# Jiraiya812/Fast-CU-Decision-HEVC

Hardware: AMD Instinct MI355X
Metric: CTUs/sec (RDO decision only) at 4K all-intra (higher is better)
Workload: dtype int32+f64

## Files before the change

fast-cu-decision-hevc_amd/csrc/fcu_engine.h:

```cpp
#pragma once
#include <stdint.h>
#include <string.h>
#include <type_traits>
#include "../../include/fcu.h"

#ifdef FCU_EMU
#include <math.h>
#include <stdio.h>
#include <stdlib.h>
#define FCU_DEV static inline
#define FCU_MEMBER inline
#define FCU_NOINLINE
#define FCU_INLINE
#define FCU_TABLE static const
static int g_emu_phase = 0, g_emu_in_phase = 0, g_emu_lane = 0, g_emu_relax = 0;
#define FCU_EMU_RELAX(on) (g_emu_relax = (on))
static inline int fcu_emu_phase_begin() { g_emu_phase++; g_emu_in_phase = 1; g_emu_lane = 0; return 0; }
static inline int fcu_emu_phase_next(int lane) { if (lane + 1 >= 64) g_emu_in_phase = 0; g_emu_lane = lane + 1; return lane + 1; }
template <class T> static inline T fcu_emu_uni(T v, int site, int line)
{
  enum { SITES = 2048, K = 32, B = 16 };
  struct Seen { int phase, first, cur, idx, n; unsigned char vals[K][B]; };
  static Seen seen[SITES];
  if (g_emu_in_phase && !g_emu_relax && sizeof(T) <= B && site < SITES) {
// ... 75 lines not shown
#define FCU_DIST_ADD(acc, v, e, i, n2) do { \
    if ((n2) >= 64) { (acc) += (uint32_t)((e) * (e)); if (((((i) - lane) + 64) & ((n2) - 1)) == 0) { FCU_WAVE_ADD(&g_S.vc_dist[v], acc); (acc) = 0; } } \
    else FCU_ATOMIC_ADD(&g_S.vc_dist[v], (uint32_t)((e) * (e))); } while (0)
#define FCU_SERIAL FCU_FOR_LANES if (lane == 0)
#if defined(FCU_PROFILE) && !defined(FCU_EMU)
#define FCU_TIC(v) const long long v = clock64()
#ifdef FCU_PROFILE_RQT
#define FCU_QTIC(v) long long v = clock64()
#define FCU_QTOC(E_, v, idx) do { if (threadIdx.x == 0) (E_).C->prof[idx] += (unsigned long long)(clock64() - v); v = clock64(); } while (0)
#define FCU_TOC(E_, v, idx) do { if ((idx) == 10 && threadIdx.x == 0) (E_).C->prof[idx] += (unsigned long long)(clock64() - v); } while (0)
#define FCU_COUNT(E_, idx, n) do { } while (0)
#elif defined(FCU_PROFILE_INTER)
#define FCU_ITOC(E_, v, idx) do { if (threadIdx.x == 0) (E_).C->prof[idx] += (unsigned long long)(clock64() - v); } while (0)
#define FCU_TOC(E_, v, idx) do { if ((idx) == 10 && threadIdx.x == 0) (E_).C->prof[idx] += (unsigned long long)(clock64() - v); } while (0)
#define FCU_COUNT(E_, idx, n) do { } while (0)
#elif defined(FCU_PROFILE_RDOQ) || defined(FCU_PROFILE_DEPTH)
#define FCU_TOC(E_, v, idx) do { if ((idx) < 11 && threadIdx.x == 0) (E_).C->prof[idx] += (unsigned long long)(clock64() - v); } while (0)
#define FCU_COUNT(E_, idx, n) do { } while (0)
#elif defined(FCU_PROFILE_RMD)
#define FCU_MTOC(E_, v, idx) do { if (threadIdx.x == 0) (E_).C->prof[idx] += (unsigned long long)(clock64() - v); } while (0)
#define FCU_TOC(E_, v, idx) do { if ((idx) < 11 && threadIdx.x == 0) (E_).C->prof[idx] += (unsigned long long)(clock64() - v); } while (0)
#define FCU_COUNT(E_, idx, n) do { } while (0)
#elif defined(FCU_PROFILE_CUSYN)
#define FCU_STOC(E_, v, idx) do { if (threadIdx.x == 0) (E_).C->prof[idx] += (unsigned long long)(clock64() - v); } while (0)
#define FCU_SPATH(E_, path) do { if (threadIdx.x == 0) (E_).C->prof[15] += 1ull << (21 * (path)); } while (0)
#define FCU_S7_COEFF(E_, v, comp) do { if (g_S.prof_s7 == 1) FCU_STOC(E_, v, (comp) ? 14 : 13); } while (0)
#define FCU_TOC(E_, v, idx) do { if ((idx) < 11 && threadIdx.x == 0) (E_).C->prof[idx] += (unsigned long long)(clock64() - v); } while (0)
#define FCU_COUNT(E_, idx, n) do { } while (0)
#elif defined(FCU_PROFILE_PIX)
#define FCU_PTIC(v) long long v = clock64()
// ... 33 lines not shown
#endif

#include "fcu_tables.h"

struct HotTables { uint32_t bin[256]; uint16_t scan[3][16]; uint8_t scan_cg8[3][4]; uint8_t ctx_ind_map4x4[16]; uint8_t group_idx[32];
                   uint64_t scan4_nib[3], map4_nib; uint32_t cnt_bits[4]; };
#ifdef FCU_EMU
static HotTables g_hot;
#else
__shared__ HotTables g_hot;
#endif

#if defined(FCU_PROFILE_RQT) && !defined(FCU_EMU)
#define FCU_RTIC(v) long long v = clock64()
#define FCU_RTOC(P_, v, idx) do { if (!SER && threadIdx.x == 0) { ((Chain *)((char *)&(P_) - __builtin_offsetof(Chain, p)))->prof[idx] += (unsigned long long)(clock64() - v); v = clock64(); } } while (0)
#elif defined(FCU_PROFILE_RDOQ) && !defined(FCU_EMU)
#define FCU_RTIC(v) long long v = clock64()
#define FCU_RTOC(P_, v, idx) do { if ((FCU_PROFILE_RDOQ + 0) == 2 ? (!SER && threadIdx.x == 0) : SER) { ((Chain *)((char *)&(P_) - __builtin_offsetof(Chain, p)))->prof[idx] += (unsigned long long)(clock64() - v); v = clock64(); } } while (0)
#else
#define FCU_RTIC(v) do { } while (0)
#define FCU_RTOC(P_, v, idx) do { } while (0)
#endif
namespace fcu {

enum { CTU = 64, MAXDEPTH = 3, NPART = 256, LOG2_MAXTU = 5, LOG2_MINTU = 2, TU_MAXDEPTH_INTRA = 3 };
enum { SIZE_2Nx2N = 0, SIZE_2NxN = 1, SIZE_Nx2N = 2, SIZE_NxN = 3, SIZE_2NxnU = 4, SIZE_2NxnD = 5, SIZE_nLx2N = 6, SIZE_nRx2N = 7, SIZE_NONE = 8, MODE_INTER = 0, MODE_INTRA = 1, MODE_NONE = 2 };
enum { SLICE_I = 0, SLICE_P = 1 };
enum { PLANAR = 0, DC = 1, HOR = 10, VER = 26, DM_CHROMA = 36 };
enum { CTX_SPLIT = 0, CTX_PARTSIZE = 3, CTX_INTRA_LUMA = 4, CTX_CHROMA_PRED = 5, CTX_CBF_LUMA = 6, CTX_CBF_CHROMA = 11,
       CTX_SUBDIV = 16, CTX_SIGCG = 19, CTX_SIG = 23, CTX_LASTX = 67, CTX_LASTY = 97, CTX_ONE = 127, CTX_ABS = 151,
       CTX_TSKIP = 157, NCTX_INTRA = 160,
       CTX_SKIP = 160, CTX_MERGE_FLAG = 163, CTX_MERGE_IDX = 164, CTX_PRED_MODE = 165, CTX_PARTSIZE1 = 166, CTX_MVD = 169,
       CTX_REF = 171, CTX_MVP_IDX = 173, CTX_ROOT_CBF = 174, NCTX = 176 };
enum { CI_CURR_BEST = 0, CI_NEXT_BEST, CI_TEMP_BEST, CI_CHROMA_INTRA, CI_QT_TRAFO_TEST, CI_QT_TRAFO_ROOT, CI_NUM };
enum { MEMO_K = 6, MEMO_POOL = 6144 + 1536 + 384 + 96 };
enum { MAXVC = 20, MAXLC = 16, POOL = 5120 };
// ... 297 lines not shown
  return first + offset;
}
FCU_DEV int coef_remain_bins(uint32_t symbol, uint32_t rparam)
{
  int code = (int)symbol;
  if (code < (3 << rparam)) return (int)(((uint32_t)code >> rparam) + 1) + (int)rparam;
  uint32_t length = rparam;
  code -= 3 << rparam;
  while (code >= (1 << length)) code -= 1 << (length++);
  return (int)(3 + length + 1 - rparam) + (int)length;
}
#ifdef FCU_EMU
enum { WALK_RDOQ_CALLS, WALK_RDOQ_TOP_IS_GROUP0, WALK_RDOQ_AHEAD_GROUPS, WALK_RDOQ_ONLY_GROUP0, WALK_RDOQ_ONLY_LAST_GROUP, WALK_RDOQ_ALL_ZERO,
       WALK_BITS_CALLS, WALK_BITS_ONE_EMPTY_RUN_BETWEEN, WALK_BITS_SECOND_ROUND, WALK_N };
enum { SMALL_TS_WINNER, SMALL_ALL_ZERO, SMALL_BATCH_OVER_16, SMALL_CHROMA_4X4, SMALL_N };
extern "C" { __attribute__((weak)) unsigned long long fcu_emu_walk_cnt[WALK_N]; __attribute__((weak)) unsigned long long fcu_emu_small_cnt[SMALL_N]; }
#define FCU_SMALL_COUNT(i, n) (fcu_emu_small_cnt[i] += (unsigned long long)(n))
static const int32_t *g_emu_lscan_lo = nullptr, *g_emu_lscan_hi = nullptr;
#define FCU_WALK_COUNT(i, n) (fcu_emu_walk_cnt[i] += (unsigned long long)(n))
#define FCU_CHECK_LSCAN(p) FCU_CHECK((const int32_t *)(p) >= g_emu_lscan_lo && (const int32_t *)(p) < g_emu_lscan_hi)
#else
#define FCU_WALK_COUNT(i, n) do { } while (0)
#define FCU_SMALL_COUNT(i, n) do { } while (0)
#define FCU_CHECK_LSCAN(p) do { } while (0)
#endif
template <int SER>
FCU_DEV FCU_INLINE void code_coeff_body(int c, const int16_t *coef, int st, int last, int log2, int comp, int scanType, int tsFlag, const Params &P_, int16_t *absCoeff)
{
  if (SER) { c = FCU_UNI(c); coef = FCU_UNI(coef); last = FCU_UNI(last); scanType = FCU_UNI(scanType); tsFlag = FCU_UNI(tsFlag); absCoeff = FCU_UNI(absCoeff); }
  const Params &P = *FCU_UNI(&P_);
  st = FCU_UNI(st); log2 = FCU_UNI(log2); comp = FCU_UNI(comp);
  FCU_IN_LDS(absCoeff);
  const FCU_HBM int16_t *coefg = (const FCU_HBM int16_t *)coef;
  const int ch = comp ? 1 : 0, N = 1 << log2; int n2 = N * N;
  if (last < 0 && st == 1 && n2 >= 64) {
    int q = (n2 >> 6) - 1;
    for (; q >= 0; q--) {
      uint32_t w[32];
// ... 558 lines not shown
  }
#endif
  return rdoq_finish<SER>(cb, P, srcg, dstg, recg, cgg, st, log2, ch, scanType, cbfCtx, scan, scanCG, cgflag, cgLastScanPos, lastScanPos, baseCost, blockUncodedCost, lambda);
}

#ifdef FCU_EMU
template <class T> struct LaneVar {
  T v[64];
  LaneVar() { for (int i = 0; i < 64; i++) v[i] = T(); }
  void set(int lane, T x) { v[lane] = x; }
  T own(int lane) const { return v[lane]; }
  T get(int k) const { return v[k]; }
  void put(int k, T x) { v[k] = x; }
  T from(int src) const { return v[src & 63]; }
};
FCU_DEV uint32_t lane_mask16(const LaneVar<int> &f) { uint32_t m = 0; for (int k = 0; k < 16; k++) m |= (uint32_t)(f.v[k] != 0) << k; return m; }
#else
#if defined(__HIP_DEVICE_COMPILE__)
#define FCU_READLANE(v, k) __builtin_amdgcn_readlane((v), (k))
#define FCU_WRITELANE(val_, k_, old_) (((int)threadIdx.x == (k_)) ? (val_) : (old_))
#define FCU_BALLOT(p) __builtin_amdgcn_ballot_w64(p)
#define FCU_PERMUTE(v, src) __builtin_amdgcn_ds_bpermute((src) << 2, (v))
#else
#define FCU_READLANE(v, k) (v)
#define FCU_WRITELANE(val_, k_, old_) (val_)
#define FCU_BALLOT(p) ((unsigned long long)(p))
#define FCU_PERMUTE(v, src) (v)
#endif
template <class T> struct LaneVar;
template <> struct LaneVar<int> {
  int r = 0;
  __device__ void set(int, int x) { r = x; }
  __device__ int own(int) const { return r; }
  __device__ int get(int k) const { return FCU_READLANE(r, k); }
  __device__ void put(int k, int x) { r = FCU_WRITELANE(x, k, r); }
  __device__ int from(int src) const { return FCU_PERMUTE(r, src); }
};
template <> struct LaneVar<double> {
  double r = 0;
  __device__ void set(int, double x) { r = x; }
  __device__ double own(int) const { return r; }
  __device__ double get(int k) const
  { union { double d; int i[2]; } u; u.d = r; u.i[0] = FCU_READLANE(u.i[0], k); u.i[1] = FCU_READLANE(u.i[1], k); return u.d; }
  __device__ void put(int k, double x)
  { union { double d; int i[2]; } u, w; u.d = r; w.d = x; u.i[0] = FCU_WRITELANE(w.i[0], k, u.i[0]); u.i[1] = FCU_WRITELANE(w.i[1], k, u.i[1]); r = u.d; }
};
__device__ inline uint32_t lane_mask16(const LaneVar<int> &f) { return (uint32_t)FCU_BALLOT(f.r != 0) & 0xffffu; }
#endif

#ifndef FCU_WAVE_RDOQ_MIN_LOG2
#define FCU_WAVE_RDOQ_MIN_LOG2 2
#endif
FCU_DEV FCU_NOINLINE void rdoq_wave(int c, const int32_t *src, int16_t *dst, int topNZ, int log2, int comp, int scanType, int cbfCtx, const Params &P_, RdoqRec *rec, double *costCGSig)
{
  const Params &P = *FCU_UNI(&P_);
  c = FCU_UNI(c); src = FCU_UNI(src); dst = FCU_UNI(dst); topNZ = FCU_UNI(topNZ); log2 = FCU_UNI(log2); comp = FCU_UNI(comp);
  scanType = FCU_UNI(scanType); cbfCtx = FCU_UNI(cbfCtx); rec = FCU_UNI(rec); costCGSig = FCU_UNI(costCGSig);
  if (topNZ < 0) { FCU_SERIAL { g_S.rw_abs = 0; g_S.rw_lsp = -1; } return; }
  const FCU_HBM int32_t *srcg = (const FCU_HBM int32_t *)src; FCU_HBM int16_t *dstg = (FCU_HBM int16_t *)dst;
  FCU_HBM RdoqRec *recg = (FCU_HBM RdoqRec *)rec; FCU_HBM double *cgg = (FCU_HBM double *)costCGSig;
  auto cb = [&](int ctx, int bin) -> int { return (int)FCU_EST[ctx * 2 + bin]; };
  const int ch = comp ? 1 : 0, N = 1 << log2, n2 = N * N;
  const int qp = comp ? P.qp_c : P.qp;
  const int qbits = rdoq_qbits(log2, qp);
  const double lambda = P.rdoq_lambda[comp];
  const double errScale = P.err_scale[ch][log2 - 2];
  const uint16_t *scan = log2 == 2 ? &g_hot.scan[scanType][0] : k_scan + k_scan_off[scanType * 4 + log2 - 2];
  const uint8_t *scanCG = log2 <= 3 ? g_hot.scan_cg8[log2 == 2 ? 0 : scanType] : k_scan_cg + k_scan_cg_off[scanType * 4 + log2 - 2];
  const int wg = N >> 2, firstSig = first_sig_ctx(log2, scanType, ch);
  const int sigOff = CTX_SIG + (ch ? 28 : 0), cgBase = CTX_SIGCG + (ch ? 2 : 0);
  const uint64_t scan4 = g_hot.scan4_nib[scanType], map4 = g_hot.map4_nib;
  const int cgTop = topNZ >> 4;
  uint64_t cgflag = 0;
  int cgLastScanPos = -1; uint32_t ctxSet = 0; int c1 = 1, c2 = 0;
  double baseCost = 0, blockUncodedCost = 0;
  int lastScanPos = -1; uint32_t c1Idx = 0, c2Idx = 0, goRice = 0;
  int g10 = 0, g10Ctx = -1;
  for (int cg = (n2 >> 4) - 1; cg > cgTop; cg -= 4) {
    LaneVar<double> t0;
    FCU_FOR_LANES { const int g = cg - (lane >> 4); if (g > cgTop) { const double err = (double)iabs(srcg[g * 16 + (lane & 15)]); t0.set(lane, err * err * errScale); } }
    for (int j = 0; j < 4 && cg - j > cgTop; j++)
      for (int k = 15; k >= 0; k--) blockUncodedCost += t0.get(j * 16 + k);
  }
  baseCost = blockUncodedCost;
  LaneVar<int> vCgBlk, vNext;
  LaneVar<double> vCgSig;
  FCU_FOR_LANES { if (lane <= cgTop) vCgBlk.set(lane, scanCG[lane]); if (lane < 16) vNext.set(lane, srcg[cgTop * 16 + lane]); }
  for (int cgScanPos = cgTop; cgScanPos >= 0; cgScanPos--) {
    const int cgBlk = vCgBlk.get(cgScanPos), cgy = cgBlk / wg, cgx = cgBlk - cgy * wg;
    const int sigBase = sigOff + firstSig + ((!ch && (cgx + cgy) > 0) ? 3 : 0);
    const uint32_t cntBits = g_hot.cnt_bits[pattern_sig_ctx(cgflag, cgx, cgy, wg)];
    LaneVar<int> vLd, vMax, vSb0, vSb1, vUp, vDn, vSd, vDu, vLv, vCand;
    LaneVar<double> vC0, vCs, vCc;
    FCU_FOR_LANES {
      if (lane < 16) {
        const int posInCG = lane, scanPos = cgScanPos * 16 + posInCG;
        const int32_t levelDouble = iabs(vNext.own(lane));
        if (cgScanPos > 0) vNext.set(lane, srcg[scanPos - 16]);
        uint32_t maxAbsLevel = (uint32_t)((levelDouble + ((int32_t)1 << (qbits - 1))) >> qbits);
        if (maxAbsLevel > 32767u) maxAbsLevel = 32767u;
        const double err = (double)levelDouble;
        const double c0 = err * err * errScale;
        const int p4 = (int)((scan4 >> (4 * posInCG)) & 15);
        int ctxSig;
        if (log2 == 2) ctxSig = sigOff + (p4 ? (int)((map4 >> (4 * p4)) & 15) : 0);
        else if (scanPos == 0) ctxSig = sigOff;
        else ctxSig = sigBase + (int)((cntBits >> (2 * p4)) & 3);
        const int sbit0 = cb(ctxSig, 0), sbit1 = cb(ctxSig, 1);
        vLd.set(lane, levelDouble); vMax.set(lane, (int)maxAbsLevel); vSb0.set(lane, sbit0); vSb1.set(lane, sbit1);
        vC0.set(lane, c0); vCand.set(lane, maxAbsLevel != 0);
        const double cs = lambda * (double)sbit0;
        vCs.set(lane, cs); vCc.set(lane, c0 + cs); vSd.set(lane, sbit1 - sbit0); vDu.set(lane, (int32_t)(levelDouble >> (qbits - 8)));
        vUp.set(lane, 0); vDn.set(lane, 0); vLv.set(lane, 0);
      }
    }
    const uint32_t cand = lane_mask16(vCand);
    double rdSigCost = 0, rdSigCost0 = 0, rdCodedLevelandDist = 0, rdUncodedDist = 0; int nnzBeforePos0 = 0;
    double cgSig = 0;
    for (int posInCG = 15; posInCG >= 0; posInCG--) {
      const int scanPos = cgScanPos * 16 + posInCG;
      const int isCand = (int)((cand >> posInCG) & 1);
      double c0 = vC0.get(posInCG), cc = 0, cs = 0;
      blockUncodedCost += c0;
      uint32_t level = 0;
      if (isCand && lastScanPos < 0) {
        lastScanPos = scanPos;
        ctxSet = (uint32_t)((ch ? 4 : 0) + ((!ch && (scanPos >> 4) > 0) ? 2 : 0));
        cgLastScanPos = cgScanPos;
      }
      if (lastScanPos >= 0) {
        const int oneCtx = CTX_ONE + 4 * (int)ctxSet + c1;
        if (oneCtx != g10Ctx) { g10 = cb(oneCtx, 0); g10Ctx = oneCtx; }
        if (!isCand) {
          cs = vCs.get(posInCG); cc = vCc.get(posInCG);
          vUp.put(posInCG, g10);
          baseCost += cc;
          rdSigCost += cs;
          if (posInCG == 0) rdSigCost0 = cs;
          continue;
        }
        const int32_t levelDouble = vLd.get(posInCG); const uint32_t maxAbsLevel = (uint32_t)vMax.get(posInCG);
        const int sbit0 = vSb0.get(posInCG), sbit1 = vSb1.get(posInCG);
        auto cbs = [&](int, int bin) -> int { return bin ? sbit1 : sbit0; };
        int sdel = 0, rup, rdn = 0;
        const int absCtx = CTX_ABS + (int)ctxSet + c2;
        LevelBits lb; lb.g10 = g10; lb.g11 = cb(oneCtx, 1); lb.g20 = cb(absCtx, 0); lb.g21 = cb(absCtx, 1);
        int rateHi = 0, rateLo = 0;
        if (scanPos == lastScanPos)
          level = coded_level(cbs, lambda, &cc, &c0, &cs, levelDouble, maxAbsLevel,
                              0, lb, goRice, c1Idx, c2Idx, qbits, errScale, 1, &rateHi, &rateLo);
        else {
          level = coded_level(cbs, lambda, &cc, &c0, &cs, levelDouble, maxAbsLevel,
                              0, lb, goRice, c1Idx, c2Idx, qbits, errScale, 0, &rateHi, &rateLo);
          sdel = sbit1 - sbit0;
        }
        if (level > 0) {
          if (level == maxAbsLevel) {
            rup = ic_rate(lb, level + 1, goRice, c1Idx, c2Idx) - rateHi;
            rdn = (maxAbsLevel > 1 ? rateLo : ic_rate(lb, 0, goRice, c1Idx, c2Idx)) - rateHi;
          } else {
            rup = rateHi - rateLo;
            rdn = ic_rate(lb, level - 1, goRice, c1Idx, c2Idx) - rateLo;
          }
        } else rup = lb.g10;
        vCc.put(posInCG, cc); vCs.put(posInCG, cs); vC0.put(posInCG, c0); vUp.put(posInCG, rup); vDn.put(posInCG, rdn); vSd.put(posInCG, sdel);
        vDu.put(posInCG, (int32_t)((levelDouble - ((int32_t)level << qbits)) >> (qbits - 8)));
        baseCost += cc;
        const uint32_t baseLevel = (c1Idx < 8) ? (2 + (c2Idx < 1)) : 1;
        if (level >= baseLevel) { if (level > 3u * (1u << goRice)) goRice = goRice + 1 < 4 ? goRice + 1 : 4; }
        if (level >= 1) c1Idx++;
        if (level > 1) { c1 = 0; c2 += (c2 < 2); c2Idx++; }
        else if (c1 < 3 && c1 > 0 && level) c1++;
      } else baseCost += c0;
      vLv.put(posInCG, (int)level);
      rdSigCost += cs;
      if (posInCG == 0) rdSigCost0 = cs;
      if (level) {
        cgflag |= 1ull << cgBlk;
        rdCodedLevelandDist += cc - cs;
        rdUncodedDist += c0;
        if (posInCG != 0) nnzBeforePos0++;
      }
    }
    if (lastScanPos >= 0 && cgScanPos > 0) {
      ctxSet = (uint32_t)((ch ? 4 : 0) + ((!ch && (cgScanPos - 1) > 0) ? 2 : 0) + (c1 == 0));
      c1 = 1; c2 = 0; c1Idx = 0; c2Idx = 0; goRice = 0;
    }
    int zeroed = 0;
    if (cgLastScanPos >= 0) {
// ... 2 lines not shown
          const int ctxSig = cgBase + sig_cg_ctx(cgflag, cgx, cgy, wg);
          baseCost += lambda * (double)cb(ctxSig, 0) - rdSigCost;
          cgSig = lambda * (double)cb(ctxSig, 0);
        } else if (cgScanPos < cgLastScanPos) {
          if (nnzBeforePos0 == 0) { baseCost -= rdSigCost0; rdSigCost -= rdSigCost0; }
          double costZeroCG = baseCost;
          const int ctxSig = cgBase + sig_cg_ctx(cgflag, cgx, cgy, wg);
          baseCost += lambda * (double)cb(ctxSig, 1);
          costZeroCG += lambda * (double)cb(ctxSig, 0);
          cgSig = lambda * (double)cb(ctxSig, 1);
          costZeroCG += rdUncodedDist; costZeroCG -= rdCodedLevelandDist; costZeroCG -= rdSigCost;
          if (costZeroCG < baseCost) {
            cgflag &= ~(1ull << cgBlk); baseCost = costZeroCG;
            cgSig = lambda * (double)cb(ctxSig, 0);
            zeroed = 1;
          }
        }
      } else cgflag |= 1ull << cgBlk;
    }
    const int keepsLevel = (int)((cgflag >> cgBlk) & 1);
    FCU_FOR_LANES {
      if (lane < 16) {
        const int sp = cgScanPos * 16 + lane;
        if (keepsLevel) {
          RdoqRec r; r.cc = vCc.own(lane); r.cs = vCs.own(lane); r.c0 = vC0.own(lane); r.up = vUp.own(lane); r.dn = vDn.own(lane); r.sd = vSd.own(lane); r.du = vDu.own(lane);
          recg[sp] = r;
        }
        dstg[sp] = (int16_t)(zeroed ? 0 : vLv.own(lane));
      }
      if (lane == 0) cgg[cgScanPos] = cgSig;
    }
    vCgSig.put(cgScanPos, cgSig);
  }
  if (lastScanPos < 0) { FCU_SERIAL { g_S.rw_abs = 0; g_S.rw_lsp = -1; } return; }
  int bestLastIdxP1 = 0;
  {
    double bestCost = blockUncodedCost + lambda * (double)cb(cbfCtx, 0);
    baseCost += lambda * (double)cb(cbfCtx, 1);
    const int lcc = log2 - 2, loff = ch ? 0 : (lcc * 3 + ((lcc + 1) >> 2)), lsh = ch ? lcc : ((lcc + 3) >> 2);
    const int lbx = CTX_LASTX + (ch ? 15 : 0) + loff, lby = CTX_LASTY + (ch ? 15 : 0) + loff, lgmax = g_hot.group_idx[N - 1];
    int foundLast = 0;
    for (int cgScanPos = cgLastScanPos; cgScanPos >= 0 && !foundLast; cgScanPos--) {
      const int cgBlk = vCgBlk.get(cgScanPos);
      baseCost -= vCgSig.get(cgScanPos);
      if (!((cgflag >> cgBlk) & 1)) continue;
      const int top = (cgScanPos * 16 + 15 > lastScanPos) ? lastScanPos - cgScanPos * 16 : 15;
      LaneVar<int> wLv; LaneVar<double> wCs, wCc, wC0, wCl;
      FCU_FOR_LANES {
        if (lane <= top) {
          const int scanPos = cgScanPos * 16 + lane;
          const int lv = dstg[scanPos];
          const RdoqRec q = recg[scanPos];
          wLv.set(lane, lv); wCs.set(lane, q.cs); wCc.set(lane, q.cc); wC0.set(lane, q.c0);
          double costLast = 0;
          if (lv) {
            const int blk = scan[scanPos];
            const int py = blk >> log2, px = blk - (py << log2);
            const int ax = scanType == 2 ? py : px, ay = scanType == 2 ? px : py;
            const int gx = g_hot.group_idx[ax], gy = g_hot.group_idx[ay];
            int bxs = 0, bys = 0;
            for (int k = 0; k < gx; k++) bxs += cb(lbx + (k >> lsh), 1);
            if (gx < lgmax) bxs += cb(lbx + (gx >> lsh), 0);
            for (int k = 0; k < gy; k++) bys += cb(lby + (k >> lsh), 1);
            if (gy < lgmax) bys += cb(lby + (gy >> lsh), 0);
            double r = (double)(bxs + bys);
            if (gx > 3) r += 32768.0 * (double)((gx - 2) >> 1);
            if (gy > 3) r += 32768.0 * (double)((gy - 2) >> 1);
            costLast = lambda * r;
          }
          wCl.set(lane, costLast);
        }
      }
      for (int posInCG = top; posInCG >= 0; posInCG--) {
        const int lv = wLv.get(posInCG); const double curCs = wCs.get(posInCG);
        if (lv) {
          const double totalCost = baseCost + wCl.get(posInCG) - curCs;
          if (totalCost < bestCost) { bestLastIdxP1 = cgScanPos * 16 + posInCG + 1; bestCost = totalCost; }
          if (lv > 1) { foundLast = 1; break; }
          baseCost -= wCc.get(posInCG); baseCost += wC0.get(posInCG);
        } else baseCost -= curCs;
      }
    }
  }
  FCU_SERIAL { g_S.rw_abs = 0; }
  FCU_FOR_LANES {
    uint32_t acc = 0;
    for (int sp = lane; sp <= lastScanPos; sp += 64) {
      if (sp < bestLastIdxP1) { const int lv = dstg[sp]; acc += (uint32_t)lv; dstg[sp] = (int16_t)((srcg[sp] < 0) ? -lv : lv); }
      else dstg[sp] = 0;
    }
    FCU_WAVE_ADD((uint32_t *)&g_S.rw_abs, acc);
  }
  FCU_SERIAL {
    const int absSum = g_S.rw_abs;
    rdoq_sign_hiding(P, srcg, dstg, recg, 1, ch, bestLastIdxP1, absSum);
    int last = bestLastIdxP1 - 1;
    while (last >= 0 && dstg[last] == 0) last--;
    g_S.rw_lsp = last;
  }
}

FCU_DEV int use_filtered_ref(int mode, int log2, int isLuma)
{
  if (!isLuma || mode == DC) return 0;
  const int d1 = iabs(mode - HOR), d2 = iabs(mode - VER);
  return (d1 < d2 ? d1 : d2) > k_filter_thr[log2 - 2];
}
FCU_DEV int pred_pixel(const uint8_t *ref, int log2, int mode, int isLuma, int dc, int x, int y)
{
  const int N = 1 << log2;
  const uint8_t *corner = ref + 2 * N;
  if (mode == PLANAR)
    return ((N - 1 - x) * corner[-1 - y] + (x + 1) * corner[1 + N] + (N - 1 - y) * corner[1 + x] + (y + 1) * corner[-1 - N] + N) >> (log2 + 1);
  if (mode == DC) {
// ... 2188 lines not shown
```

fast-cu-decision-hevc_amd/csrc/fcu_inter.h:

```cpp

struct Pu { int addr, ox, oy, w, h; };
FCU_DEV int pu_count(int ps) { return ps == SIZE_2Nx2N ? 1 : (ps == SIZE_NxN ? 4 : 2); }
FCU_TABLE uint32_t k_pu_geom[8][4] = { { 0x04400, 0x04400, 0x04400, 0x04400 }, { 0x02400, 0x82420, 0x00000, 0x00000 }, { 0x04200, 0x44202, 0x00000, 0x00000 }, { 0x02200, 0x42202, 0x82220, 0xc2222 }, { 0x01400, 0x23410, 0x00000, 0x00000 }, { 0x03400, 0xa1430, 0x00000, 0x00000 }, { 0x04100, 0x14301, 0x00000, 0x00000 }, { 0x04300, 0x54103, 0x00000, 0x00000 } };
FCU_DEV Pu pu_geom(int depth, int ps, int pu)
{
  const int s = CTU >> depth, n = NPART >> (2 * depth);
  const uint32_t e = k_pu_geom[ps][pu];
  Pu g; g.ox = (int)((e & 7) * s) >> 2; g.oy = (int)(((e >> 4) & 7) * s) >> 2; g.w = (int)(((e >> 8) & 7) * s) >> 2; g.h = (int)(((e >> 12) & 7) * s) >> 2;
  g.addr = (int)(((e >> 16) & 15) * n) >> 4;
  return g;
}
FCU_DEV int pu_covers(int n, int ps, int pu, int i)
{
  if (ps == SIZE_2Nx2N) return 1;
  if (ps == SIZE_2NxN) return (i >= (n >> 1)) == (pu != 0);
  if (ps == SIZE_Nx2N) return ((i / (n >> 2)) & 1) == pu;
  if (ps == SIZE_NxN) return i / (n >> 2) == pu;
  const int lx = part_x(i), ly = part_y(i), s = n == 256 ? 64 : (n == 64 ? 32 : (n == 16 ? 16 : 8)), q = s >> 2;
  if (ps == SIZE_2NxnU) return (ly >= q) == (pu != 0);
  if (ps == SIZE_2NxnD) return (ly >= s - q) == (pu != 0);
  if (ps == SIZE_nLx2N) return (lx >= q) == (pu != 0);
  return (lx >= s - q) == (pu != 0);
}
FCU_DEV void pu_set_motion(CuObj *cu, int ps, int pu, int lane, int mvx, int mvy, int ref)
// ... 793 lines not shown
      auto put = [&](int k, int32_t t) {
        const int sp = iscan[k]; const int32_t ld = level_double(t, qscale, qbits);
        G->p_lscan[o + sp] = ld;
        if (level_nonzero(ld, qbits)) FCU_ATOMIC_MAX(&g_S.iv_top[v], sp);
      };
      if (v & 1) { for (int k = lane; k < n2; k += 64) put(k, (int32_t)G->p_resi[boff[comp] + k] << (15 - 8 - l2)); }
      else by_log2(l2, [&](auto L) { constexpr int LG = decltype(L)::value; RowCache<(1 << LG), int32_t> rc; for (int k = lane; k < n2; k += 64) put(k, fwd2<LG>(rc, G->p_tmp + boff[comp], 0, k)); });
    }
  }
  FCU_QTOC(E, q_, 0);
  const int waveY = FCU_UNI((int)(log2 >= 3 && P.rdoq)), waveC = FCU_UNI((int)(NC && lc >= 3 && P.rdoq));
  for (int v = 0; v < 6; v += 2) {
    const int comp = v >> 1;
    if (!(comp ? waveC : waveY) || comp >= ncomp) continue;
    const int cbfCtx = (comp == 0 && trMode == 0) ? EST_ROOT_CBF : qt_cbf_ctx(tu, comp);
    rdoq_wave(CAB_GOON, G->p_lscan + voff(v), G->p_qscan + voff(v), FCU_UNI(g_S.iv_top[v]), bl2[comp], comp ? 1 : 0, 0, cbfCtx, P, G->r_rec + voff(v), G->r_cg + v * 64);
    FCU_SERIAL { g_S.iv_abs[v] = g_S.rw_abs; g_S.iv_lsp[v] = g_S.rw_lsp; }
  }
  for (int ch = 0; ch < (NC ? 2 : 1); ch++) {
    if (ch ? waveC : waveY) continue;
    FCU_FOR_LANES {
      if (lane < 6 && vok(lane) && ((lane >> 1) != 0) == (ch != 0)) {
        const int comp = lane >> 1, l2 = bl2[comp], o = voff(lane);
        const int cbfCtx = (comp == 0 && trMode == 0) ? EST_ROOT_CBF : qt_cbf_ctx(tu, comp);
        const RdoqOut r = ((lane & 1) ? P.rdoq_ts : P.rdoq)
          ? rdoq<0, 1>(CAB_GOON, G->p_lscan + o, G->p_qscan + o, 1, g_S.iv_top[lane], l2, comp ? 1 : 0, 0, cbfCtx, P, G->r_rec + o, G->r_cg + lane * 64, lane)
          : quant_plain(G->p_lscan + o, G->p_qscan + o, 1, g_S.iv_top[lane], l2, comp ? 1 : 0, P);
        g_S.iv_abs[lane] = r.abs_sum; g_S.iv_lsp[lane] = r.last;
      }
    }
// ... 301 lines not shown
```

Baseline: 20680.

## Keep 8x8 RDOQ state in wave registers and parallelize sign-hiding tail

For transform blocks up to 8x8, the wave RDOQ path now keeps all coefficients and per-position records in lane registers across coefficient groups instead of writing them to global/shared pools and reading them back. The last-position search, abs-sum reduction and sign-data-hiding search are done in-wave (ballot masks, lane-parallel cost evaluation) rather than by a serial single-lane routine. Memory round-trips and serial-lane work are cut in exchange for more register pressure, plus a large new code path that must match the reference sign-hiding semantics. Profiling and emulator checks are added behind macros.

```diff
diff --git a/fast-cu-decision-hevc_amd/csrc/fcu_engine.h b/fast-cu-decision-hevc_amd/csrc/fcu_engine.h
--- a/fast-cu-decision-hevc_amd/csrc/fcu_engine.h
+++ b/fast-cu-decision-hevc_amd/csrc/fcu_engine.h
@@ -113,6 +113,9 @@
 #define FCU_ITOC(E_, v, idx) do { if (threadIdx.x == 0) (E_).C->prof[idx] += (unsigned long long)(clock64() - v); } while (0)
 #define FCU_TOC(E_, v, idx) do { if ((idx) == 10 && threadIdx.x == 0) (E_).C->prof[idx] += (unsigned long long)(clock64() - v); } while (0)
 #define FCU_COUNT(E_, idx, n) do { } while (0)
+#elif defined(FCU_PROFILE_RDOQ) && (FCU_PROFILE_RDOQ + 0) == 3
+#define FCU_TOC(E_, v, idx) do { if ((idx) == 10 && threadIdx.x == 0) (E_).C->prof[idx] += (unsigned long long)(clock64() - v); } while (0)
+#define FCU_COUNT(E_, idx, n) do { } while (0)
 #elif defined(FCU_PROFILE_RDOQ) || defined(FCU_PROFILE_DEPTH)
 #define FCU_TOC(E_, v, idx) do { if ((idx) < 11 && threadIdx.x == 0) (E_).C->prof[idx] += (unsigned long long)(clock64() - v); } while (0)
 #define FCU_COUNT(E_, idx, n) do { } while (0)
@@ -176,12 +179,20 @@
 #if defined(FCU_PROFILE_RQT) && !defined(FCU_EMU)
 #define FCU_RTIC(v) long long v = clock64()
 #define FCU_RTOC(P_, v, idx) do { if (!SER && threadIdx.x == 0) { ((Chain *)((char *)&(P_) - __builtin_offsetof(Chain, p)))->prof[idx] += (unsigned long long)(clock64() - v); v = clock64(); } } while (0)
-#elif defined(FCU_PROFILE_RDOQ) && !defined(FCU_EMU)
+#elif defined(FCU_PROFILE_RDOQ) && (FCU_PROFILE_RDOQ + 0) != 3 && !defined(FCU_EMU)
 #define FCU_RTIC(v) long long v = clock64()
 #define FCU_RTOC(P_, v, idx) do { if ((FCU_PROFILE_RDOQ + 0) == 2 ? (!SER && threadIdx.x == 0) : SER) { ((Chain *)((char *)&(P_) - __builtin_offsetof(Chain, p)))->prof[idx] += (unsigned long long)(clock64() - v); v = clock64(); } } while (0)
 #else
 #define FCU_RTIC(v) do { } while (0)
 #define FCU_RTOC(P_, v, idx) do { } while (0)
+#endif
+#if defined(FCU_PROFILE_RDOQ) && (FCU_PROFILE_RDOQ + 0) == 3 && !defined(FCU_EMU)
+#define FCU_WTIC(v) long long v = clock64()
+#define FCU_WTOC(P_, v, t, log2) do { if (threadIdx.x == 0) { const int s_ = (t) * 3 + ((log2) >= 4 ? 2 : (log2) - 2); \
+    ((Chain *)((char *)&(P_) - __builtin_offsetof(Chain, p)))->prof[s_ + (s_ >= 10)] += (unsigned long long)(clock64() - v); } v = clock64(); } while (0)
+#else
+#define FCU_WTIC(v) do { } while (0)
+#define FCU_WTOC(P_, v, t, log2) do { } while (0)
 #endif
 namespace fcu {
 
@@ -509,14 +520,19 @@
 enum { WALK_RDOQ_CALLS, WALK_RDOQ_TOP_IS_GROUP0, WALK_RDOQ_AHEAD_GROUPS, WALK_RDOQ_ONLY_GROUP0, WALK_RDOQ_ONLY_LAST_GROUP, WALK_RDOQ_ALL_ZERO,
        WALK_BITS_CALLS, WALK_BITS_ONE_EMPTY_RUN_BETWEEN, WALK_BITS_SECOND_ROUND, WALK_N };
 enum { SMALL_TS_WINNER, SMALL_ALL_ZERO, SMALL_BATCH_OVER_16, SMALL_CHROMA_4X4, SMALL_N };
-extern "C" { __attribute__((weak)) unsigned long long fcu_emu_walk_cnt[WALK_N]; __attribute__((weak)) unsigned long long fcu_emu_small_cnt[SMALL_N]; }
+enum { TAIL_SH_4X4, TAIL_SH_8X8_LOW, TAIL_SH_BIG, TAIL_SH_TIE, TAIL_SH_CLEARED_LAST, TAIL_LAST_ZERO, TAIL_CG_ZEROED_8X8, TAIL_TOP_IN_GROUP0_8X8,
+       TAIL_CHROMA, TAIL_INTER, TAIL_SH_NO_FINITE, TAIL_N };
+extern "C" { __attribute__((weak)) unsigned long long fcu_emu_walk_cnt[WALK_N]; __attribute__((weak)) unsigned long long fcu_emu_small_cnt[SMALL_N];
+             __attribute__((weak)) unsigned long long fcu_emu_tail_cnt[TAIL_N]; }
 #define FCU_SMALL_COUNT(i, n) (fcu_emu_small_cnt[i] += (unsigned long long)(n))
+#define FCU_TAIL_COUNT(i, n) (fcu_emu_tail_cnt[i] += (unsigned long long)(n))
 static const int32_t *g_emu_lscan_lo = nullptr, *g_emu_lscan_hi = nullptr;
 #define FCU_WALK_COUNT(i, n) (fcu_emu_walk_cnt[i] += (unsigned long long)(n))
 #define FCU_CHECK_LSCAN(p) FCU_CHECK((const int32_t *)(p) >= g_emu_lscan_lo && (const int32_t *)(p) < g_emu_lscan_hi)
 #else
 #define FCU_WALK_COUNT(i, n) do { } while (0)
 #define FCU_SMALL_COUNT(i, n) do { } while (0)
+#define FCU_TAIL_COUNT(i, n) do { } while (0)
 #define FCU_CHECK_LSCAN(p) do { } while (0)
 #endif
 template <int SER>
@@ -1105,7 +1121,9 @@
   void put(int k, T x) { v[k] = x; }
   T from(int src) const { return v[src & 63]; }
 };
-FCU_DEV uint32_t lane_mask16(const LaneVar<int> &f) { uint32_t m = 0; for (int k = 0; k < 16; k++) m |= (uint32_t)(f.v[k] != 0) << k; return m; }
+FCU_DEV uint32_t lane_nz16(const LaneVar<int> &f, int lb) { uint32_t m = 0; for (int k = 0; k < 16; k++) m |= (uint32_t)(f.v[lb + k] != 0) << k; return m; }
+FCU_DEV uint32_t lane_odd16(const LaneVar<int> &f, int lb) { uint32_t m = 0; for (int k = 0; k < 16; k++) m |= (uint32_t)(f.v[lb + k] & 1) << k; return m; }
+FCU_DEV int lane_sum(const LaneVar<int> &f) { uint32_t s = 0; for (int k = 0; k < 64; k++) s += (uint32_t)f.v[k]; return (int)s; }
 #else
 #if defined(__HIP_DEVICE_COMPILE__)
 #define FCU_READLANE(v, k) __builtin_amdgcn_readlane((v), (k))
@@ -1136,7 +1154,9 @@
   __device__ void put(int k, double x)
   { union { double d; int i[2]; } u, w; u.d = r; w.d = x; u.i[0] = FCU_WRITELANE(w.i[0], k, u.i[0]); u.i[1] = FCU_WRITELANE(w.i[1], k, u.i[1]); r = u.d; }
 };
-__device__ inline uint32_t lane_mask16(const LaneVar<int> &f) { return (uint32_t)FCU_BALLOT(f.r != 0) & 0xffffu; }
+__device__ inline uint32_t lane_nz16(const LaneVar<int> &f, int lb) { return (uint32_t)(FCU_BALLOT(f.r != 0) >> lb) & 0xffffu; }
+__device__ inline uint32_t lane_odd16(const LaneVar<int> &f, int lb) { return (uint32_t)(FCU_BALLOT((f.r & 1) != 0) >> lb) & 0xffffu; }
+__device__ inline int lane_sum(const LaneVar<int> &f) { return (int)fcu_wave_sum((uint32_t)f.r); }
 #endif
 
 #ifndef FCU_WAVE_RDOQ_MIN_LOG2
@@ -1162,11 +1182,20 @@
   const int sigOff = CTX_SIG + (ch ? 28 : 0), cgBase = CTX_SIGCG + (ch ? 2 : 0);
   const uint64_t scan4 = g_hot.scan4_nib[scanType], map4 = g_hot.map4_nib;
   const int cgTop = topNZ >> 4;
+  const int inRegs = log2 <= 3;
+  const int nStore = (cgTop + 1) << 4;
+#ifdef FCU_EMU_CHECK_RDOQ_TAIL
+  const int toPools = 1;
+#else
+  const int toPools = !inRegs;
+#endif
+  FCU_TAIL_COUNT(TAIL_CHROMA, ch); FCU_TAIL_COUNT(TAIL_TOP_IN_GROUP0_8X8, log2 == 3 && cgTop == 0);
   uint64_t cgflag = 0;
   int cgLastScanPos = -1; uint32_t ctxSet = 0; int c1 = 1, c2 = 0;
   double baseCost = 0, blockUncodedCost = 0;
   int lastScanPos = -1; uint32_t c1Idx = 0, c2Idx = 0, goRice = 0;
   int g10 = 0, g10Ctx = -1;
+  FCU_WTIC(wt_);
   for (int cg = (n2 >> 4) - 1; cg > cgTop; cg -= 4) {
     LaneVar<double> t0;
     FCU_FOR_LANES { const int g = cg - (lane >> 4); if (g > cgTop) { const double err = (double)iabs(srcg[g * 16 + (lane & 15)]); t0.set(lane, err * err * errScale); } }
@@ -1176,18 +1205,24 @@
   baseCost = blockUncodedCost;
   LaneVar<int> vCgBlk, vNext;
   LaneVar<double> vCgSig;
-  FCU_FOR_LANES { if (lane <= cgTop) vCgBlk.set(lane, scanCG[lane]); if (lane < 16) vNext.set(lane, srcg[cgTop * 16 + lane]); }
+  FCU_FOR_LANES_REG {
+    if (lane <= cgTop) vCgBlk.set(lane, scanCG[lane]);
+    if (inRegs) { if (lane < nStore) vNext.set(lane, srcg[lane]); }
+    else if (lane < 16) vNext.set(lane, srcg[cgTop * 16 + lane]);
+  }
+  FCU_WTOC(P, wt_, 0, log2);
+  LaneVar<int> vLd, vMax, vSb0, vSb1, vUp, vDn, vSd, vDu, vLv, vCand;
+  LaneVar<double> vC0, vCs, vCc;
   for (int cgScanPos = cgTop; cgScanPos >= 0; cgScanPos--) {
+    const int lb = inRegs ? cgScanPos << 4 : 0;
     const int cgBlk = vCgBlk.get(cgScanPos), cgy = cgBlk / wg, cgx = cgBlk - cgy * wg;
     const int sigBase = sigOff + firstSig + ((!ch && (cgx + cgy) > 0) ? 3 : 0);
     const uint32_t cntBits = g_hot.cnt_bits[pattern_sig_ctx(cgflag, cgx, cgy, wg)];
-    LaneVar<int> vLd, vMax, vSb0, vSb1, vUp, vDn, vSd, vDu, vLv, vCand;
-    LaneVar<double> vC0, vCs, vCc;
-    FCU_FOR_LANES {
-      if (lane < 16) {
-        const int posInCG = lane, scanPos = cgScanPos * 16 + posInCG;
+    FCU_FOR_LANES_REG {
+      if ((unsigned)(lane - lb) < 16u) {
+        const int posInCG = lane - lb, scanPos = cgScanPos * 16 + posInCG;
         const int32_t levelDouble = iabs(vNext.own(lane));
-        if (cgScanPos > 0) vNext.set(lane, srcg[scanPos - 16]);
+        if (!inRegs && cgScanPos > 0) vNext.set(lane, srcg[scanPos - 16]);
         uint32_t maxAbsLevel = (uint32_t)((levelDouble + ((int32_t)1 << (qbits - 1))) >> qbits);
         if (maxAbsLevel > 32767u) maxAbsLevel = 32767u;
         const double err = (double)levelDouble;
@@ -1205,13 +1240,13 @@
         vUp.set(lane, 0); vDn.set(lane, 0); vLv.set(lane, 0);
       }
     }
-    const uint32_t cand = lane_mask16(vCand);
+    const uint32_t cand = lane_nz16(vCand, lb);
     double rdSigCost = 0, rdSigCost0 = 0, rdCodedLevelandDist = 0, rdUncodedDist = 0; int nnzBeforePos0 = 0;
     double cgSig = 0;
     for (int posInCG = 15; posInCG >= 0; posInCG--) {
-      const int scanPos = cgScanPos * 16 + posInCG;
+      const int scanPos = cgScanPos * 16 + posInCG, ln = lb + posInCG;
       const int isCand = (int)((cand >> posInCG) & 1);
-      double c0 = vC0.get(posInCG), cc = 0, cs = 0;
+      double c0 = vC0.get(ln), cc = 0, cs = 0;
       blockUncodedCost += c0;
       uint32_t level = 0;
       if (isCand && lastScanPos < 0) {
@@ -1223,39 +1258,39 @@
         const int oneCtx = CTX_ONE + 4 * (int)ctxSet + c1;
         if (oneCtx != g10Ctx) { g10 = cb(oneCtx, 0); g10Ctx = oneCtx; }
         if (!isCand) {
-          cs = vCs.get(posInCG); cc = vCc.get(posInCG);
-          vUp.put(posInCG, g10);
+          cs = vCs.get(ln); cc = vCc.get(ln);
+          vUp.put(ln, g10);
           baseCost += cc;
           rdSigCost += cs;
           if (posInCG == 0) rdSigCost0 = cs;
           continue;
         }
-        const int32_t levelDouble = vLd.get(posInCG); const uint32_t maxAbsLevel = (uint32_t)vMax.get(posInCG);
-        const int sbit0 = vSb0.get(posInCG), sbit1 = vSb1.get(posInCG);
+        const int32_t levelDouble = vLd.get(ln); const uint32_t maxAbsLevel = (uint32_t)vMax.get(ln);
+        const int sbit0 = vSb0.get(ln), sbit1 = vSb1.get(ln);
         auto cbs = [&](int, int bin) -> int { return bin ? sbit1 : sbit0; };
         int sdel = 0, rup, rdn = 0;
         const int absCtx = CTX_ABS + (int)ctxSet + c2;
-        LevelBits lb; lb.g10 = g10; lb.g11 = cb(oneCtx, 1); lb.g20 = cb(absCtx, 0); lb.g21 = cb(absCtx, 1);
+        LevelBits lb4; lb4.g10 = g10; lb4.g11 = cb(oneCtx, 1); lb4.g20 = cb(absCtx, 0); lb4.g21 = cb(absCtx, 1);
         int rateHi = 0, rateLo = 0;
         if (scanPos == lastScanPos)
           level = coded_level(cbs, lambda, &cc, &c0, &cs, levelDouble, maxAbsLevel,
-                              0, lb, goRice, c1Idx, c2Idx, qbits, errScale, 1, &rateHi, &rateLo);
+                              0, lb4, goRice, c1Idx, c2Idx, qbits, errScale, 1, &rateHi, &rateLo);
         else {
           level = coded_level(cbs, lambda, &cc, &c0, &cs, levelDouble, maxAbsLevel,
-                              0, lb, goRice, c1Idx, c2Idx, qbits, errScale, 0, &rateHi, &rateLo);
+                              0, lb4, goRice, c1Idx, c2Idx, qbits, errScale, 0, &rateHi, &rateLo);
           sdel = sbit1 - sbit0;
         }
         if (level > 0) {
           if (level == maxAbsLevel) {
-            rup = ic_rate(lb, level + 1, goRice, c1Idx, c2Idx) - rateHi;
-            rdn = (maxAbsLevel > 1 ? rateLo : ic_rate(lb, 0, goRice, c1Idx, c2Idx)) - rateHi;
+            rup = ic_rate(lb4, level + 1, goRice, c1Idx, c2Idx) - rateHi;
+            rdn = (maxAbsLevel > 1 ? rateLo : ic_rate(lb4, 0, goRice, c1Idx, c2Idx)) - rateHi;
           } else {
             rup = rateHi - rateLo;
-            rdn = ic_rate(lb, level - 1, goRice, c1Idx, c2Idx) - rateLo;
+            rdn = ic_rate(lb4, level - 1, goRice, c1Idx, c2Idx) - rateLo;
           }
-        } else rup = lb.g10;
-        vCc.put(posInCG, cc); vCs.put(posInCG, cs); vC0.put(posInCG, c0); vUp.put(posInCG, rup); vDn.put(posInCG, rdn); vSd.put(posInCG, sdel);
-        vDu.put(posInCG, (int32_t)((levelDouble - ((int32_t)level << qbits)) >> (qbits - 8)));
+        } else rup = lb4.g10;
+        vCc.put(ln, cc); vCs.put(ln, cs); vC0.put(ln, c0); vUp.put(ln, rup); vDn.put(ln, rdn); vSd.put(ln, sdel);
+        vDu.put(ln, (int32_t)((levelDouble - ((int32_t)level << qbits)) >> (qbits - 8)));
         baseCost += cc;
         const uint32_t baseLevel = (c1Idx < 8) ? (2 + (c2Idx < 1)) : 1;
         if (level >= baseLevel) { if (level > 3u * (1u << goRice)) goRice = goRice + 1 < 4 ? goRice + 1 : 4; }
@@ -1263,7 +1298,7 @@
         if (level > 1) { c1 = 0; c2 += (c2 < 2); c2Idx++; }
         else if (c1 < 3 && c1 > 0 && level) c1++;
       } else baseCost += c0;
-      vLv.put(posInCG, (int)level);
+      vLv.put(ln, (int)level);
       rdSigCost += cs;
       if (posInCG == 0) rdSigCost0 = cs;
       if (level) {
@@ -1296,90 +1331,198 @@
             cgflag &= ~(1ull << cgBlk); baseCost = costZeroCG;
             cgSig = lambda * (double)cb(ctxSig, 0);
             zeroed = 1;
+            FCU_TAIL_COUNT(TAIL_CG_ZEROED_8X8, log2 == 3);
           }
         }
       } else cgflag |= 1ull << cgBlk;
     }
-    const int keepsLevel = (int)((cgflag >> cgBlk) & 1);
-    FCU_FOR_LANES {
-      if (lane < 16) {
-        const int sp = cgScanPos * 16 + lane;
-        if (keepsLevel) {
-          RdoqRec r; r.cc = vCc.own(lane); r.cs = vCs.own(lane); r.c0 = vC0.own(lane); r.up = vUp.own(lane); r.dn = vDn.own(lane); r.sd = vSd.own(lane); r.du = vDu.own(lane);
-          recg[sp] = r;
-        }
-        dstg[sp] = (int16_t)(zeroed ? 0 : vLv.own(lane));
-      }
-      if (lane == 0) cgg[cgScanPos] = cgSig;
+    if (zeroed) FCU_FOR_LANES_REG { if ((unsigned)(lane - lb) < 16u) vLv.set(lane, 0); }
+    if (toPools) {
+      const int keepsLevel = (int)((cgflag >> cgBlk) & 1);
+      FCU_FOR_LANES {
+        if ((unsigned)(lane - lb) < 16u) {
+          const int sp = cgScanPos * 16 + lane - lb;
+          if (keepsLevel) {
+            RdoqRec r; r.cc = vCc.own(lane); r.cs = vCs.own(lane); r.c0 = vC0.own(lane); r.up = vUp.own(lane); r.dn = vDn.own(lane); r.sd = vSd.own(lane); r.du = vDu.own(lane);
+            recg[sp] = r;
+          }
+          dstg[sp] = (int16_t)vLv.own(lane);
+        }
+        if (lane == 0) cgg[cgScanPos] = cgSig;
+      }
     }
     vCgSig.put(cgScanPos, cgSig);
   }
-  if (lastScanPos < 0) { FCU_SERIAL { g_S.rw_abs = 0; g_S.rw_lsp = -1; } return; }
+  FCU_WTOC(P, wt_, 1, log2);
+  if (lastScanPos < 0) {
+    FCU_FOR_LANES { if (inRegs && lane < nStore) dstg[lane] = 0; if (lane == 0) { g_S.rw_abs = 0; g_S.rw_lsp = -1; } }
+    return;
+  }
+#ifdef FCU_EMU_CHECK_RDOQ_TAIL
+  int16_t chkLv[1024]; const double chkBase = baseCost; int chkSkip = 0;
+  for (int sp = 0; sp < nStore; sp++) chkLv[sp] = dstg[sp];
+#endif
   int bestLastIdxP1 = 0;
   {
     double bestCost = blockUncodedCost + lambda * (double)cb(cbfCtx, 0);
     baseCost += lambda * (double)cb(cbfCtx, 1);
     const int lcc = log2 - 2, loff = ch ? 0 : (lcc * 3 + ((lcc + 1) >> 2)), lsh = ch ? lcc : ((lcc + 3) >> 2);
     const int lbx = CTX_LASTX + (ch ? 15 : 0) + loff, lby = CTX_LASTY + (ch ? 15 : 0) + loff, lgmax = g_hot.group_idx[N - 1];
+    auto costOfLast = [&](int scanPos) -> double {
+      const int blk = scan[scanPos];
+      const int py = blk >> log2, px = blk - (py << log2);
+      const int ax = scanType == 2 ? py : px, ay = scanType == 2 ? px : py;
+      const int gx = g_hot.group_idx[ax], gy = g_hot.group_idx[ay];
+      int bxs = 0, bys = 0;
+      for (int k = 0; k < gx; k++) bxs += cb(lbx + (k >> lsh), 1);
+      if (gx < lgmax) bxs += cb(lbx + (gx >> lsh), 0);
+      for (int k = 0; k < gy; k++) bys += cb(lby + (k >> lsh), 1);
+      if (gy < lgmax) bys += cb(lby + (gy >> lsh), 0);
+      double r = (double)(bxs + bys);
+      if (gx > 3) r += 32768.0 * (double)((gx - 2) >> 1);
+      if (gy > 3) r += 32768.0 * (double)((gy - 2) >> 1);
+      return lambda * r;
+    };
+    LaneVar<double> wCl;
+    if (inRegs) FCU_FOR_LANES_REG { if (lane <= lastScanPos) wCl.set(lane, vLv.own(lane) ? costOfLast(lane) : 0.0); }
     int foundLast = 0;
     for (int cgScanPos = cgLastScanPos; cgScanPos >= 0 && !foundLast; cgScanPos--) {
+      const int lb = inRegs ? cgScanPos << 4 : 0;
       const int cgBlk = vCgBlk.get(cgScanPos);
       baseCost -= vCgSig.get(cgScanPos);
       if (!((cgflag >> cgBlk) & 1)) continue;
       const int top = (cgScanPos * 16 + 15 > lastScanPos) ? lastScanPos - cgScanPos * 16 : 15;
-      LaneVar<int> wLv; LaneVar<double> wCs, wCc, wC0, wCl;
-      FCU_FOR_LANES {
+      if (!inRegs) FCU_FOR_LANES_REG {
         if (lane <= top) {
           const int scanPos = cgScanPos * 16 + lane;
           const int lv = dstg[scanPos];
           const RdoqRec q = recg[scanPos];
-          wLv.set(lane, lv); wCs.set(lane, q.cs); wCc.set(lane, q.cc); wC0.set(lane, q.c0);
-          double costLast = 0;
-          if (lv) {
-            const int blk = scan[scanPos];
-            const int py = blk >> log2, px = blk - (py << log2);
-            const int ax = scanType == 2 ? py : px, ay = scanType == 2 ? px : py;
-            const int gx = g_hot.group_idx[ax], gy = g_hot.group_idx[ay];
-            int bxs = 0, bys = 0;
-            for (int k = 0; k < gx; k++) bxs += cb(lbx + (k >> lsh), 1);
-            if (gx < lgmax) bxs += cb(lbx + (gx >> lsh), 0);
-            for (int k = 0; k < gy; k++) bys += cb(lby + (k >> lsh), 1);
-            if (gy < lgmax) bys += cb(lby + (gy >> lsh), 0);
-            double r = (double)(bxs + bys);
-            if (gx > 3) r += 32768.0 * (double)((gx - 2) >> 1);
-            if (gy > 3) r += 32768.0 * (double)((gy - 2) >> 1);
-            costLast = lambda * r;
-          }
-          wCl.set(lane, costLast);
+          vLv.set(lane, lv); vCs.set(lane, q.cs); vCc.set(lane, q.cc); vC0.set(lane, q.c0);
+          wCl.set(lane, lv ? costOfLast(scanPos) : 0.0);
         }
       }
       for (int posInCG = top; posInCG >= 0; posInCG--) {
-        const int lv = wLv.get(posInCG); const double curCs = wCs.get(posInCG);
+        const int ln = lb + posInCG;
+        const int lv = vLv.get(ln); const double curCs = vCs.get(ln);
         if (lv) {
-          const double totalCost = baseCost + wCl.get(posInCG) - curCs;
+          const double totalCost = baseCost + wCl.get(ln) - curCs;
           if (totalCost < bestCost) { bestLastIdxP1 = cgScanPos * 16 + posInCG + 1; bestCost = totalCost; }
           if (lv > 1) { foundLast = 1; break; }
-          baseCost -= wCc.get(posInCG); baseCost += wC0.get(posInCG);
+          baseCost -= vCc.get(ln); baseCost += vC0.get(ln);
         } else baseCost -= curCs;
       }
     }
   }
-  FCU_SERIAL { g_S.rw_abs = 0; }
-  FCU_FOR_LANES {
+  FCU_TAIL_COUNT(TAIL_LAST_ZERO, bestLastIdxP1 == 0);
+  FCU_WTOC(P, wt_, 2, log2);
+  LaneVar<int> vAcc;
+  if (inRegs) FCU_FOR_LANES_REG {
+    const int lv = lane < bestLastIdxP1 ? vLv.own(lane) : 0;
+    vAcc.set(lane, lv); vLv.set(lane, vNext.own(lane) < 0 ? -lv : lv);
+  }
+  else FCU_FOR_LANES {
     uint32_t acc = 0;
     for (int sp = lane; sp <= lastScanPos; sp += 64) {
       if (sp < bestLastIdxP1) { const int lv = dstg[sp]; acc += (uint32_t)lv; dstg[sp] = (int16_t)((srcg[sp] < 0) ? -lv : lv); }
       else dstg[sp] = 0;
     }
-    FCU_WAVE_ADD((uint32_t *)&g_S.rw_abs, acc);
-  }
-  FCU_SERIAL {
-    const int absSum = g_S.rw_abs;
-    rdoq_sign_hiding(P, srcg, dstg, recg, 1, ch, bestLastIdxP1, absSum);
-    int last = bestLastIdxP1 - 1;
-    while (last >= 0 && dstg[last] == 0) last--;
-    g_S.rw_lsp = last;
-  }
+    vAcc.set(lane, (int)acc);
+  }
+  const int absSum = lane_sum(vAcc);
+  FCU_WTOC(P, wt_, 3, log2);
+  int last = bestLastIdxP1 - 1;
+  if (P.sign_hiding && absSum >= 2) {
+    const long long rdFactor = P.rd_factor[ch], kInf = 0x7fffffffffffffffLL;
+    int lastCG = -1;
+    for (int subSet = (bestLastIdxP1 - 1) >> 4; subSet >= 0; subSet--) {
+      if (!((cgflag >> vCgBlk.get(subSet)) & 1)) continue;
+      const int lb = inRegs ? subSet << 4 : 0, subPos = subSet << 4;
+      if (!inRegs) FCU_FOR_LANES_REG {
+        if (lane < 16) {
+          const RdoqRec q = recg[subPos + lane];
+          vLv.set(lane, dstg[subPos + lane]); vNext.set(lane, srcg[subPos + lane]);
+          vUp.set(lane, q.up); vDn.set(lane, q.dn); vSd.set(lane, q.sd); vDu.set(lane, q.du);
+        }
+      }
+      const uint32_t nzMask = lane_nz16(vLv, lb);
+      if (!nzMask) continue;
+      const int lastNZ = 31 - __builtin_clz(nzMask), firstNZ = __builtin_ctz(nzMask);
+      if (lastCG == -1) lastCG = 1;
+      if (lastNZ - firstNZ >= 4) {
+        const uint32_t signbit = vLv.get(lb + firstNZ) < 0 ? 1 : 0;
+        if (signbit != (uint32_t)(__builtin_popcount(lane_odd16(vLv, lb)) & 1)) {
+          const int nTop = lastCG == 1 ? lastNZ : 15;
+          LaneVar<int> vCostLo, vCostHi, vChg;
+          FCU_FOR_LANES_REG {
+            const int n = lane - lb;
+            long long curCost = kInf; int curChange = 0;
+            if (n >= 0 && n <= nTop) {
+              const int lv = vLv.own(lane), du = vDu.own(lane), up = vUp.own(lane), dn = vDn.own(lane), sd = vSd.own(lane);
+              if (lv != 0) {
+                const long long costUp = rdFactor * (-du) + up;
+                long long costDown = rdFactor * (du) + dn - ((iabs(lv) == 1) ? sd : 0);
+                if (lastCG == 1 && lastNZ == n && iabs(lv) == 1) costDown -= (4 << 15);
+                if (costUp < costDown) { curCost = costUp; curChange = 1; }
+                else { curChange = -1; if (n == firstNZ && iabs(lv) == 1) curCost = kInf; else curCost = costDown; }
+              } else {
+                curCost = rdFactor * (-(long long)(iabs(du))) + (1 << 15) + up + sd;
+                curChange = 1;
+                if (n < firstNZ) { const uint32_t thissign = vNext.own(lane) >= 0 ? 0 : 1; if (thissign != signbit) curCost = kInf; }
+              }
+            }
+            vCostLo.set(lane, (int)(uint32_t)(unsigned long long)curCost); vCostHi.set(lane, (int)(curCost >> 32)); vChg.set(lane, curChange);
+          }
+          long long minCostInc = kInf; int minN = -1;
+          for (int n = nTop; n >= 0; --n) {
+            const long long curCost = (long long)(((unsigned long long)(uint32_t)vCostHi.get(lb + n) << 32) | (uint32_t)vCostLo.get(lb + n));
+            if (curCost < minCostInc) { minCostInc = curCost; minN = n; }
+          }
+          if (minN >= 0) {
+#ifdef FCU_EMU
+            { int same = 0;
+              for (int n = nTop; n >= 0; --n) same += vCostHi.get(lb + n) == vCostHi.get(lb + minN) && vCostLo.get(lb + n) == vCostLo.get(lb + minN);
+              FCU_TAIL_COUNT(TAIL_SH_TIE, same > 1); }
+#endif
+            const int old = vLv.get(lb + minN); int finalChange = vChg.get(lb + minN);
+            if (old == 32767 || old == -32768) finalChange = -1;
+            const int nv = (int)(int16_t)(vNext.get(lb + minN) >= 0 ? old + finalChange : old - finalChange);
+            vLv.put(lb + minN, nv);
+            if (!inRegs) FCU_FOR_LANES_REG { if (lane == 0) dstg[subPos + minN] = (int16_t)nv; }
+            FCU_TAIL_COUNT(TAIL_SH_4X4, log2 == 2); FCU_TAIL_COUNT(TAIL_SH_8X8_LOW, log2 == 3 && lastCG == 0); FCU_TAIL_COUNT(TAIL_SH_BIG, log2 >= 4);
+          } else {
+            FCU_TAIL_COUNT(TAIL_SH_NO_FINITE, 1);
+#ifdef FCU_EMU_CHECK_RDOQ_TAIL
+            chkSkip = 1;
+#endif
+          }
+        }
+      }
+      if (lastCG == 1) {
+        const uint32_t nzNow = lane_nz16(vLv, lb);
+        last = subPos + 31 - __builtin_clz(nzNow);
+        FCU_TAIL_COUNT(TAIL_SH_CLEARED_LAST, last != bestLastIdxP1 - 1);
+        lastCG = 0;
+      }
+    }
+  }
+  if (inRegs) {
+    FCU_FOR_LANES { if (lane < nStore) dstg[lane] = (int16_t)vLv.own(lane); if (lane == 0) { g_S.rw_abs = absSum; g_S.rw_lsp = last; } }
+  } else {
+    FCU_SERIAL { g_S.rw_abs = absSum; g_S.rw_lsp = last; }
+  }
+  FCU_WTOC(P, wt_, 4, log2);
+#ifdef FCU_EMU_CHECK_RDOQ_TAIL
+  if (!chkSkip) {
+    const RdoqOut o = rdoq_finish<1>(cb, P, srcg, chkLv, recg, cgg, 1, log2, ch, scanType, cbfCtx, scan, scanCG, cgflag, cgLastScanPos, lastScanPos, chkBase, blockUncodedCost, lambda);
+    int bad = o.abs_sum != g_S.rw_abs || o.last != g_S.rw_lsp;
+    for (int sp = 0; sp < nStore; sp++) bad |= chkLv[sp] != dstg[sp];
+    if (bad) {
+      fprintf(stderr, "FCU_EMU_CHECK_RDOQ_TAIL: rdoq_wave differs from rdoq_finish (log2 %d comp %d scan %d topNZ %d: abs %d / %d, last %d / %d)\n",
+              log2, comp, scanType, topNZ, g_S.rw_abs, o.abs_sum, g_S.rw_lsp, o.last);
+      abort();
+    }
+  }
+#endif
 }
 
 FCU_DEV int use_filtered_ref(int mode, int log2, int isLuma)
diff --git a/fast-cu-decision-hevc_amd/csrc/fcu_inter.h b/fast-cu-decision-hevc_amd/csrc/fcu_inter.h
--- a/fast-cu-decision-hevc_amd/csrc/fcu_inter.h
+++ b/fast-cu-decision-hevc_amd/csrc/fcu_inter.h
@@ -831,6 +831,7 @@
     const int comp = v >> 1;
     if (!(comp ? waveC : waveY) || comp >= ncomp) continue;
     const int cbfCtx = (comp == 0 && trMode == 0) ? EST_ROOT_CBF : qt_cbf_ctx(tu, comp);
+    FCU_TAIL_COUNT(TAIL_INTER, 1);
     rdoq_wave(CAB_GOON, G->p_lscan + voff(v), G->p_qscan + voff(v), FCU_UNI(g_S.iv_top[v]), bl2[comp], comp ? 1 : 0, 0, cbfCtx, P, G->r_rec + voff(v), G->r_cg + v * 64);
     FCU_SERIAL { g_S.iv_abs[v] = g_S.rw_abs; g_S.iv_lsp[v] = g_S.rw_lsp; }
   }
```

After: 21280, median of 6. 1.03x the previous value.
